# leggedrobotics/open3d_slam_private

Measured on AMD Instinct MI355X. Metric: ICP iterations/sec (scan-to-map), higher is better.
Workload: dtype f32

## Files before the change

open3d_slam_private_amd/csrc/host_loop.hpp:

```cpp
#pragma once


static reg_status check_ready(reg_handle* h, bool need_prepared) {
    if (!h) return REG_BAD_ARGUMENT;
    if (!h->device_ok) return REG_DEVICE_ERROR;
    if (h->m == 0) {
        h->err = "no reference set (reg_set_target)";
        return REG_NOT_CONFIGURED;
    }
    if (h->n == 0) {
        h->err = "no reading set (reg_set_source)";
        return REG_NOT_CONFIGURED;
    }
    if (need_prepared && !h->prepared) {
        h->err = "reg_prepare has not been called for this reading";
        return REG_NOT_CONFIGURED;
    }
    return REG_OK;
}

static reg_status prepare_rowmajor(reg_handle* h, const float* T_init_row, const float* c_override = nullptr,
                                   int64_t n_global = 0, const IterState* init_state = nullptr) {
    reg_status s = check_ready(h, false);
    if (s != REG_OK) return s;
// ... 27 lines not shown
    }
    pmark("centroid");
    PrepArgs pa;
    pa.sums = sums;
    pa.sums_to_clear = sums_next;
    pa.n = n_global > 0 ? n_global : n;
    pa.c_ref = make_float3(h->c_ref[0], h->c_ref[1], h->c_ref[2]);
    std::memcpy(pa.T_init.m, T_init_row, 64);
    pa.centre = p2pl ? 1 : 0;
    pa.use_override = c_override ? 1 : 0;
    pa.c_override = c_override ? make_float3(c_override[0], c_override[1], c_override[2]) : make_float3(0.f, 0.f, 0.f);
    pa.out = h->s_prep.as<PrepState>();
    pa.host_out = h->d_prep_host;
    h->prep_pending = true;
    StateInit si;
    si.dst = nullptr;
    if (init_state) {
        si.init = *init_state;
        si.dst = h->i_iter.as<IterState>();
    } else {
        std::memset(&si.init, 0, sizeof(si.init));
    }
    k_prepare_source<<<grid_for(n), 256, 0, h->stream>>>(
        h->s_raw.as<float>(), h->s_stride, (p2pl && h->has_snrm) ? h->s_nrm_raw.as<float>() : nullptr, h->s_nstride, n, pa,
        p2pl ? 1 : 0, h->perm, h->s_xyz.as<float4>(), (p2pl && h->has_snrm) ? h->s_nrm.as<float4>() : nullptr,
        h->i_hint.as<uint8_t>(), h->i_hist.as<uint32_t>(), h->i_acc.as<double>(), kAccRows * kSums, si,
        h->i_cache.as<float4>());
    if (h->prm.cost == REG_COST_GICP)
        k_pack_cov<<<grid_for(n), 256, 0, h->stream>>>(h->s_cov_raw.as<float>(), n, h->perm, h->s_cov.as<float4>());
    pmark("prepare_source");
    HIPCHK(h, hipGetLastError());
    h->prepared = true;
    h->match_launches = 0;
    h->have_match = false;
    h->pm_have_match = false;
    return REG_OK;
}


static reg_status build_iter_state(reg_handle* h, const float* T_row, int update, IterState* st) {
    std::memset(st, 0, sizeof(IterState));
    for (int i = 0; i < 16; ++i) {
        st->T[i] = T_row[i];
        st->Td[i] = (double)T_row[i];
    }
    st->chk = Checkers();
    st->chk.max_iter = h->prm.max_iter;
    st->chk.min_diff_rot = h->prm.min_diff_rot;
    st->chk.min_diff_trans = h->prm.min_diff_trans;
    st->chk.smooth_len = h->prm.smooth_len;
    st->chk.init(T_row);
    st->cost = h->prm.cost;
    st->fixed_iters = h->prm.fixed_iters;
    st->max_iter = h->prm.max_iter;
    st->update = update;
    st->gicp_rot_eps = h->prm.gicp_rot_eps;
    st->gicp_trans_eps = h->prm.gicp_trans_eps;
    st->gicp_stop_rule = h->prm.gicp_stop_rule;
    st->gicp_rel_fitness = h->prm.gicp_rel_fitness;
    st->gicp_rel_rmse = h->prm.gicp_rel_rmse;
    st->n_total = (float)(h->n_total_hint > 0 ? h->n_total_hint : h->n);
    st->band_lo = st->band_hi = INFINITY;
    st->limit_last = st->limit_prev = INFINITY;
    st->use_trim = (h->prm.cost == REG_COST_P2PL && h->prm.use_trimmed) ? 1 : 0;
    st->trim_ratio = h->prm.trim_ratio;
    st->band_cap = kBandCap;
// ... 27 lines not shown
    HIPCHK(h, hipEventRecord(h->ev_iter, h->stream));
    h->iter_copy_pending = true;
    return REG_OK;
}

static void prof_mark(reg_handle* h, int kind, bool start) {
    if (!h->profiling) return;
    hipEvent_t e;
    if (hipEventCreate(&e) != hipSuccess) return;
    (void)hipEventRecord(e, h->stream);
    h->prof_ev.push_back(e);
    if (start) h->prof_kind.push_back(kind);
}

template <class K, class... A>
static void launch_timed(reg_handle* h, int kind, K kernel, dim3 grid, dim3 block, A... args) {
    hipEvent_t e0 = nullptr, e1 = nullptr;
    if (!h->profiling || hipEventCreate(&e0) != hipSuccess || hipEventCreate(&e1) != hipSuccess) {
        if (e0) (void)hipEventDestroy(e0);
        hipLaunchKernelGGL(kernel, grid, block, 0, h->stream, args...);
        return;
    }
    hipExtLaunchKernelGGL(kernel, grid, block, 0, h->stream, e0, e1, 0, args...);
    h->prof_ev.push_back(e0);
    h->prof_ev.push_back(e1);
    h->prof_kind.push_back(kind);
}

static reg_status enqueue_match(reg_handle* h, bool zero_hist = false) {
    const bool trim = h->prm.cost == REG_COST_P2PL && h->prm.use_trimmed;
    if (trim && zero_hist) HIPCHK(h, hipMemsetAsync(h->i_hist.p, 0, 3 * 2048 * 4, h->stream));
    const bool fused_hist = h->dbg.match_variant == 3;
    uint32_t* hist0 = (trim && fused_hist) ? h->i_hist.as<uint32_t>() : nullptr;
    uint32_t* hist2 = trim ? h->i_hist.as<uint32_t>() + 4096 : nullptr;
    const IterState* it = h->i_iter.as<IterState>();
    if (h->dbg.match_variant == 1) {
        prof_mark(h, 0, true);
        k_match<<<h->n_blocks, 256, 0, h->stream>>>(h->s_xyz.as<float4>(), h->n, it, h->grid, h->i_pos.as<int>(),
                                                    h->i_d2.as<float>(), hist0, hist2, h->shift0);
        prof_mark(h, 0, false);
    } else {
        uint8_t* hint = h->dbg.match_variant == 2 ? nullptr : h->i_hint.as<uint8_t>();
        const int lanes = h->dbg.lanes_per_point == 4 ? 4 : (h->dbg.lanes_per_point == 2 ? 2 : 8);
        const int blocks = grid_for(h->n * lanes);
        const int tile = h->match_launches < 2 ? h->env.xcd_tile_first : h->env.xcd_tile_later;
        ++h->match_launches;
        const dim3 grid(xcd_tiled_grid(blocks, tile)), block(256);
        auto go = [&](auto kernel) {
            launch_timed(h, 0, kernel, grid, block, (const float4*)h->s_xyz.as<float4>(), h->n, it, h->grid,
                         h->i_pos.as<int>(), h->i_d2.as<float>(), hist0, hist2, hint, h->shift0, h->dbg.debug_flags, blocks,
                         h->i_cache.as<float4>(), tile);
        };
        if (lanes == 4)
            go(k_match_g8<4>);
        else if (lanes == 2)
            go(k_match_g8<2>);
        else
            go(k_match_g8<8>);
    }
    h->have_match = true;
    return REG_OK;
}

static reg_status enqueue_select(reg_handle* h) {
    uint32_t* hist0 = h->i_hist.as<uint32_t>();
    SelectState* st = h->i_state.as<SelectState>();
    const IterState* it = h->i_iter.as<IterState>();
    const int hb = std::min(h->n_blocks, 128);
    const float ratio = h->prm.trim_ratio;
    if (h->dbg.match_variant != 3)
        k_hist_level0<<<hb, 256, 0, h->stream>>>(h->i_d2.as<float>(), h->n, h->shift0, hist0, it);
    k_select_level<<<hb, 256, 0, h->stream>>>(h->i_d2.as<float>(), h->n, 1, h->shift0, ratio, hist0, hist0 + 2048,
                                              nullptr, st, it);
    k_select_level<<<hb, 256, 0, h->stream>>>(h->i_d2.as<float>(), h->n, 2, h->shift0, ratio, hist0 + 2048,
                                              hist0 + 4096, hist0, st, it);
    return REG_OK;
}

static FilterCfg make_filter_cfg(const reg_handle* h, int trim_mode);

static reg_status enqueue_linearize(reg_handle* h, bool want_w, bool limit_from_state = false) {
    float* w = want_w ? h->i_w.as<float>() : nullptr;
    const IterState* it = h->i_iter.as<IterState>();
    if (h->prm.cost == REG_COST_P2PL) {
        const FilterCfg f = make_filter_cfg(h, h->prm.use_trimmed ? (limit_from_state ? 1 : 2) : 0);
        k_linearize_p2pl<<<h->n_blocks, 256, 0, h->stream>>>(
            h->s_xyz.as<float4>(), h->has_snrm ? h->s_nrm.as<float4>() : nullptr, h->n, it, h->i_pos.as<int>(),
            h->i_d2.as<float>(), h->t_pts.as<float4>(), h->t_nrm.as<float4>(), f, h->i_state.as<SelectState>(),
            h->i_hist.as<uint32_t>() + 4096, h->i_hist.as<uint32_t>() + 2048, h->shift0, w,
            h->i_partials.as<double>(), h->i_cache.as<float4>());
    } else if (cost_is_o3d(h->prm.cost)) {
        const float3 o = make_float3(h->t_mid[0], h->t_mid[1], h->t_mid[2]);
        if (h->prm.cost == REG_COST_O3D_P2PL)
            k_linearize_o3d<REG_COST_O3D_P2PL><<<h->n_blocks, 256, 0, h->stream>>>(
                h->s_xyz.as<float4>(), h->n, it, h->i_pos.as<int>(), h->i_d2.as<float>(), h->t_nrm.as<float4>(), o, w,
                h->i_partials.as<double>());
        else
            k_linearize_o3d<REG_COST_O3D_P2P><<<h->n_blocks, 256, 0, h->stream>>>(
                h->s_xyz.as<float4>(), h->n, it, h->i_pos.as<int>(), h->i_d2.as<float>(), h->t_pts.as<float4>(), o, w,
                h->i_partials.as<double>());
        ++h->seq;
        k_reduce_update_o3d<<<1, 1024, 0, h->stream>>>(h->i_partials.as<double>(), h->n_blocks, h->i_iter.as<IterState>(),
                                                       h->d_mirror, h->seq);
        return REG_OK;
    } else {
        k_linearize_gicp<<<h->n_blocks, 256, 0, h->stream>>>(h->s_xyz.as<float4>(), h->s_cov.as<float4>(), h->n, it,
                                                             h->i_pos.as<int>(), h->i_d2.as<float>(),
                                                             h->t_pts.as<float4>(), h->t_cov.as<float4>(), w,
                                                             h->i_partials.as<double>());
    }
    ++h->seq;
    k_reduce_update<<<1, 1024, 0, h->stream>>>(h->i_partials.as<double>(), h->n_blocks, h->i_iter.as<IterState>(),
                                               h->d_mirror, h->seq, 0, nullptr, nullptr,
                                               h->prm.cost == REG_COST_P2PL ? h->i_state.as<SelectState>() : nullptr,
                                               nullptr, 0, 0, h->i_xicp.as<XicpState>());
    if (h->xicp_pending) {
        h->xicp_pending = false;
        const int blocks = (int)std::min<int64_t>(512, (h->n + 255) / 256);
        k_xicp_center<<<blocks, 256, 0, h->stream>>>(h->s_xyz.as<float4>(), h->n, h->i_iter.as<IterState>(),
                                                     h->i_pos.as<int>(), h->i_w.as<float>(), h->i_xicp.as<XicpState>());
        k_xicp_detect<<<blocks, 256, 0, h->stream>>>(h->s_xyz.as<float4>(), h->n, h->i_iter.as<IterState>(),
                                                     h->i_pos.as<int>(), h->i_w.as<float>(), h->t_nrm.as<float4>(),
                                                     h->i_xicp.as<XicpState>());
        k_reduce_update<<<1, 1024, 0, h->stream>>>(nullptr, 0, h->i_iter.as<IterState>(), h->d_mirror, h->seq, 2, nullptr,
                                                   nullptr, nullptr, nullptr, 0, 0, h->i_xicp.as<XicpState>());
    }
    return REG_OK;
}

static FilterCfg make_filter_cfg(const reg_handle* h, int trim_mode) {
    FilterCfg f;
    f.use_trim = trim_mode;
    f.use_normal = h->prm.use_surface_normal;
    f.use_maxdist = h->prm.use_max_dist_filter;
    f.debug = h->dbg.debug_flags;
    f.cos_max_angle = std::cos(h->prm.max_normal_angle);
    const float md = h->prm.outlier_max_dist;
    f.outlier_max_d2 = md * md;
    return f;
}

static inline float coherent_slack(const reg_handle* h) { return 0.25f * h->info.cell_size; }
static inline int coherent_search_grid(const reg_handle* h) { return (int)std::min<int64_t>(1024, (h->n + 31) / 32); }
static inline int coherent_queue_cap(int64_t n) { return (int)(((n + 255) / 256 + kQueues - 1) / kQueues) * 256; }

template <int G>
static void launch_fused(reg_handle* h, const FilterCfg& f, float* w, uint8_t* hint) {
    int blocks;
    if (h->dbg.debug_flags & 16) {
        blocks = grid_for(h->n * G);
        launch_timed(h, 1, k_iter_fused<G>, dim3(8 * ((blocks + 7) / 8)), dim3(256), (const float4*)h->s_xyz.as<float4>(),
                     (const float4*)(h->has_snrm ? h->s_nrm.as<float4>() : nullptr), h->n, h->i_iter.as<IterState>(), h->grid,
                     (const float4*)h->t_nrm.as<float4>(), f, h->i_pos.as<int>(), h->i_d2.as<float>(), w, hint,
                     h->i_band.as<float>(), (int)kBandCap, h->i_acc.as<double>(), blocks);
    } else {
        blocks = grid_for(h->n);
        launch_timed(h, 1, k_coh_check, dim3(8 * ((blocks + 7) / 8)), dim3(256), (const float4*)h->s_xyz.as<float4>(),
                     (const float4*)(h->has_snrm ? h->s_nrm.as<float4>() : nullptr), h->n, h->i_iter.as<IterState>(), h->grid,
                     (const float4*)h->t_nrm.as<float4>(), f, h->i_pos.as<int>(), h->i_d2.as<float>(), w,
                     (const float4*)h->i_cache.as<float4>(), h->i_queue.as<uint32_t>(), coherent_queue_cap(h->n),
// ... 127 lines not shown
    cfg.timeout_ticks = (unsigned long long)(h->env.tail_timeout_s * 1e8);
    float* w = want_w ? h->i_w.as<float>() : nullptr;
    uint8_t* hint = h->dbg.match_variant == 2 ? nullptr : h->i_hint.as<uint8_t>();
    hipEvent_t e0 = nullptr, e1 = nullptr;
    const bool timed = h->profiling && hipEventCreate(&e0) == hipSuccess && hipEventCreate(&e1) == hipSuccess;
    const bool gicp = h->prm.cost == REG_COST_GICP;
    auto args = [&](auto launch) {
        const float4* s_attr = gicp ? (const float4*)h->s_cov.as<float4>() : (const float4*)(h->has_snrm ? h->s_nrm.as<float4>() : nullptr);
        const float4* t_attr = gicp ? (const float4*)h->t_cov.as<float4>() : (const float4*)h->t_nrm.as<float4>();
        auto go = [&](auto kernel) {
            launch(kernel, dim3(pl.grid), dim3(kTailThreads), (const float4*)h->s_xyz.as<float4>(), s_attr, h->i_iter.as<IterState>(),
                   h->grid, t_attr, f, h->i_pos.as<int>(), h->i_d2.as<float>(), w, hint, h->i_cache.as<float4>(),
                   sync_cur, h->i_tail_rows.as<double>(), h->i_tail_band.as<float>(), h->d_mirror, cfg, sync_next);
        };
        if (gicp)
            go(k_tail<true>);
        else
            go(k_tail<false>);
    };
    if (timed) {
        args([&](auto k, dim3 g, dim3 b, auto... a) { hipExtLaunchKernelGGL(k, g, b, kTailLdsBytes, h->stream, e0, e1, 0, a...); });
        h->prof_ev.push_back(e0);
        h->prof_ev.push_back(e1);
        h->prof_kind.push_back(3);
    } else {
        if (e0) (void)hipEventDestroy(e0);
        args([&](auto k, dim3 g, dim3 b, auto... a) { hipLaunchKernelGGL(k, g, b, kTailLdsBytes, h->stream, a...); });
    }
    HIPCHK(h, hipGetLastError());
    h->have_match = true;
    return REG_OK;
}

static reg_status enqueue_iteration(reg_handle* h, bool want_w) {
    reg_status s = enqueue_match(h);
    if (s != REG_OK) return s;
    if (h->prm.cost == REG_COST_P2PL && h->prm.use_trimmed) {
        s = enqueue_select(h);
        if (s != REG_OK) return s;
    }
    return enqueue_linearize(h, want_w);
}

static inline unsigned long long mirror_seq(const reg_handle* h) {
    return __atomic_load_n(&h->h_mirror->seq, __ATOMIC_ACQUIRE);
}

static reg_status wait_seq(reg_handle* h, unsigned long long seq) {
    for (unsigned spins = 0;; ++spins) {
        if (mirror_seq(h) >= seq) return REG_OK;
        __builtin_ia32_pause();
        if ((spins & 0x3fff) == 0x3fff) {
            hipError_t e = hipStreamQuery(h->stream);
            if (e == hipSuccess) return REG_OK;
            if (e != hipErrorNotReady) {
                h->err = std::string("device fault while waiting for the iteration: ") + hipGetErrorString(e);
                return REG_DEVICE_ERROR;
            }
        }
    }
}

static reg_status iterate_once(reg_handle* h, const float* T_row, bool want_w) {
    reg_status s = init_iter_state(h, T_row, 0);
    if (s != REG_OK) return s;
    s = enqueue_iteration(h, want_w);
    if (s != REG_OK) return s;
    s = wait_seq(h, h->seq);
    if (s != REG_OK) return s;
// ... 517 lines not shown
    float T_start[16];
    if (p2pl)
        m4_identity(T_start);
    else
        std::memcpy(T_start, Ti, 64);
    std::memcpy(h->T_init, Ti, 64);
    IterState st0;
    reg_status s = build_iter_state(h, T_start, 1, &st0);
    if (s != REG_OK) return s;
    rmark("iter state");
    s = prepare_rowmajor(h, Ti, nullptr, 0, &st0);
    if (s != REG_OK) return s;
    rmark("prepared");
    h->profiling = h->dbg.profile_loop != 0;
    const bool event_timing = h->profiling || h->env.event_timing;
    if (event_timing) HIPCHK(h, hipEventRecord(h->ev0, h->stream));
    const auto t_loop_begin = std::chrono::steady_clock::now();
    rmark("ev0");
    const unsigned long long seq0 = h->seq;
    const int fixed = h->prm.fixed_iters;
    const int limit = sequence_limit(h->prm);
    const bool can_fuse = p2pl && h->dbg.disable_fused != 1;
    const bool trimming = p2pl && h->prm.use_trimmed && h->prm.trim_ratio != 1.0f;
    const int kGenericFirst = trimming ? 2 : (h->prm.cost == REG_COST_GICP ? std::max(1, h->env.gicp_tail_after) : 1);
    const int kAhead = h->env.lookahead;
    const HostMirror* mir = h->h_mirror;
    int generic_left = kGenericFirst;
    const bool trace = h->env.trace;
    float settle_tol = h->env.settle_tol;
    unsigned long long last_traced = 0;
    const auto t_loop0 = std::chrono::steady_clock::now();
    unsigned long long acked = seq0;
    int stalls = 0;
    const TailPlan tail_pl = ((can_fuse || h->prm.cost == REG_COST_GICP) && tail_eligible(h)) ? tail_plan(h) : TailPlan();
    const RegActiveGuard active(h->prm.device);
    std::unique_lock<std::mutex> tail_lock;
    if (tail_pl.ok && (active.alone() || h->env.tail_always)) {
        tail_lock = std::unique_lock<std::mutex>(g_tail_mutex[h->prm.device], std::try_to_lock);
    }
    const bool use_tail = tail_pl.ok && tail_lock.owns_lock();
    const int tail_min_iters = fixed > 0 ? 0 : h->env.tail_min_iters;
    const float fused_settle_tol = settle_tol;
    unsigned long long tail_seq = 0;
    bool tail_off = false;
    h->last_tail_launches = 0;
    h->last_tail_iters = 0;
    for (;;) {
        if (tail_seq) {
            for (unsigned spins = 0;; ++spins) {
                const unsigned long long m = mirror_seq(h);
                if (m >= tail_seq) break;
                if (m + 1 == tail_seq) {
                    const HostMirror::SeqRecord* rec = &mir->ring[(tail_seq - 1) % kSeqRing];
                    if (__atomic_load_n(&rec->seq, __ATOMIC_ACQUIRE) == tail_seq - 1 && (rec->done || rec->stall)) break;
                }
                __builtin_ia32_pause();
                if ((spins & 0xfff) == 0xfff) {
                    const hipError_t e = hipStreamQuery(h->stream);
                    if (e == hipSuccess) break;
                    if (e != hipErrorNotReady) {
                        h->tail_sync_dirty = true;
                        h->err = std::string("device fault while waiting for the tail kernel: ") + hipGetErrorString(e);
                        return REG_DEVICE_ERROR;
                    }
                }
            }
// ... 9 lines not shown
                return REG_DEVICE_ERROR;
            }
            if (!reported && !(mir->stall && std::max(mirror_seq(h), seq0) > acked)) acked = h->seq;
            if (h->env.coh_stats)
                fprintf(stderr, "[o3dreg] tail launch: %u iterations, %u point searches (%.2f %% of the point-iterations), stall cause %u, band records of its last iteration %d\n", words[2],
                        words[1], words[2] ? 100.0 * words[1] / ((double)words[2] * (double)h->n) : 0.0, words[3], reported ? mir->pad_nband : -1);
            if (reported) h->last_tail_iters += mir->pad3;
            if (reported && mir->stall && fixed <= 0) tail_off = true;
#if O3D_TAIL_STAMPS
            {
                unsigned long long st[24];
                (void)hipMemcpy(st, h->i_tail_sync.as<unsigned>() + (size_t)h->tail_sync_last * (kTailSyncBytes / 4) + kTailStampWord, sizeof(st),
                                 hipMemcpyDeviceToHost);
                const double it_n = std::max(1, reported ? mir->pad3 : 1);
                static const char* names[12] = {"check", "search", "epilogue", "bandrec+comps", "sum+publish+drain", "arrive+wait", "row sums",
                                                "band-stage", "band-scan", "band-rank", "band-add", "solve+update"};
                for (int wg = 0; wg < 2; ++wg) {
                    fprintf(stderr, "[o3dreg] tail stamps (us per iteration, %s workgroup):", wg ? "last" : "first");
                    for (int i = 0; i < 12; ++i) fprintf(stderr, " %s %.2f", names[i], st[12 * wg + i] * 0.01 / it_n);
                    fprintf(stderr, "\n");
                }
            }
#endif
            tail_seq = 0;
            continue;
        }
        const unsigned long long m_seq = std::max(mirror_seq(h), seq0);
        const bool any = m_seq > seq0;
        if (any && mir->done) break;
        if (any && mir->stall && m_seq > acked) {
            HIPCHK(h, hipStreamSynchronize(h->stream));
            acked = h->seq;
            generic_left = 2;
            ++stalls;
            continue;
        }
        if (trace && m_seq != last_traced) {
            last_traced = m_seq;
            float mt = 0.f, mr = 0.f;
            last_step_motion(mir, &mt, &mr);
            fprintf(stderr, "[o3dreg] seq %llu iter %d stall %d band_n %d limit %.6g prev %.6g band [%.6g, %.6g) step %.2e m %.2e rad\n",
                    m_seq - seq0, mir->iterations, mir->stall, mir->stall ? mir->band_count : mir->pad_nband, mir->limit_last, mir->limit_prev,
                    mir->band_lo, mir->band_hi, mt, mr);
        }
        acked = std::max(acked, m_seq);
        const int completed = any ? mir->iterations : 0;
        const int inflight = (int)(h->seq - acked);
        if (completed + inflight < limit && inflight < kAhead) {
            const bool tail_now = use_tail && !tail_off && completed + inflight >= tail_min_iters;
            settle_tol = tail_now ? h->env.tail_settle_tol : fused_settle_tol;
            bool settled = true;
            if (trimming) {
                settled = any && mir->limit_prev < INFINITY && mir->limit_last < INFINITY &&
                          std::fabs(mir->limit_last - mir->limit_prev) <= settle_tol * mir->limit_last;
            }
            if (settled && any && (p2pl || fixed <= 0) && (can_fuse || tail_now)) {
                float mt = 0.f, mr = 0.f;
                last_step_motion(mir, &mt, &mr);
                if (mt > h->env.settle_trans || mr > h->env.settle_rot) settled = false;
            }
            const auto tq0 = std::chrono::steady_clock::now();
            const bool go_generic = !(can_fuse || tail_now) || generic_left > 0 || !settled;
            if (go_generic) {
                s = enqueue_iteration(h, true);
                if (generic_left > 0) --generic_left;
            } else if (tail_now) {
                s = enqueue_tail(h, tail_pl, limit - (completed + inflight), true);
                tail_seq = h->seq;
                ++h->last_tail_launches;
            } else {
                int burst = fixed > 0 && !h->env.no_burst ? limit - (completed + inflight) : 1;
                for (; burst > 0 && s == REG_OK; --burst) s = enqueue_fused(h, true);
            }
            if (trace) {
                const auto tq1 = std::chrono::steady_clock::now();
                fprintf(stderr, "[o3dreg] t=%.1fus enqueue seq %llu (%s) took %.1fus; mirror at %llu\n",
                        std::chrono::duration<double, std::micro>(tq0 - t_loop0).count(), h->seq - seq0,
                        go_generic ? "generic" : (tail_now ? "tail" : "fused"), std::chrono::duration<double, std::micro>(tq1 - tq0).count(),
                        std::max(mirror_seq(h), seq0) - seq0);
            }
            if (s != REG_OK) return s;
            continue;
        }
        if (inflight == 0) break;
        s = wait_seq(h, acked + 1);
        if (s != REG_OK) return s;
        if (mirror_seq(h) <= acked) {
            if (hipStreamQuery(h->stream) == hipSuccess && mirror_seq(h) <= acked) acked = h->seq;
        }
    }
    h->last_stalls = stalls;
    rmark("loop done");
    if (event_timing) {
        HIPCHK(h, hipEventRecord(h->ev1, h->stream));
        HIPCHK(h, hipEventSynchronize(h->ev1));
        (void)hipEventElapsedTime(&res->loop_ms, h->ev0, h->ev1);
    } else {
        res->loop_ms = std::chrono::duration<float, std::milli>(std::chrono::steady_clock::now() - t_loop_begin).count();
// ... 610 lines not shown
```

open3d_slam_private_amd/csrc/host_target.hpp:

```cpp
#pragma once



struct DevBuf {
    void* p = nullptr;
    size_t cap = 0;
    hipError_t reserve(size_t bytes) {
        if (bytes <= cap) return hipSuccess;
        if (p) (void)hipFree(p);
        p = nullptr;
        cap = 0;
        hipError_t e = hipMalloc(&p, bytes ? bytes : 16);
        if (e == hipSuccess) cap = bytes;
        return e;
    }
    void release() {
        if (p) (void)hipFree(p);
        p = nullptr;
        cap = 0;
    }
    template <class T>
    T* as() const {
        return (T*)p;
    }
};

struct EnvSwitches {
    bool trace = false;
    bool event_timing = false;
    bool halo_occ = true;
    bool no_dynprune = false;
    bool no_empty_bound = false;
    bool no_burst = false;
    bool hints = false;
    bool stamps = false;
    bool coh_stats = false;
    bool tail_always = false;
    bool no_tail = false;
    int tail_wpc = 0;
    double dist_timeout_s = 30.0;
    float tail_timeout_s = 2.f;
    int xcd_tile_first = 32;
    int xcd_tile_later = 16;
    float settle_trans = 0.02f;
    float settle_rot = 4e-3f;
    int tail_min_iters = 8;
    int tail_tile = 0;
    bool no_gicp_tail = false;
    int gicp_tail_after = 1;
    float tail_settle_tol = 1.2f;
    int lookahead = 2;
    float settle_tol = 0.05f;
    float halo_ratio = 1.5f;
    float halo_rho = 0.4f;
    float reach_bins = 7.25f;
    float bin_occupancy = 8.f;
    float level_ratio = 2.0f;
    void read() {
        trace = getenv("O3D_TRACE") != nullptr;
        event_timing = getenv("O3D_EVENT_TIMING") != nullptr;
        no_burst = getenv("O3D_NO_BURST") != nullptr;
        no_dynprune = getenv("O3D_NO_DYNPRUNE") != nullptr;
        no_empty_bound = getenv("O3D_NO_EMPTY_BOUND") != nullptr;
        halo_occ = getenv("O3D_NO_HALO_OCC") == nullptr;
        hints = getenv("O3D_HINTS") != nullptr;
        stamps = getenv("O3D_STAMPS") != nullptr;
        coh_stats = getenv("O3D_COH_STATS") != nullptr;
        tail_always = getenv("O3D_TAIL_ALWAYS") != nullptr;
        no_tail = getenv("O3D_NO_TAIL") != nullptr;
        if (const char* v = getenv("O3D_TAIL_WPC")) tail_wpc = std::max(0, atoi(v));
        if (const char* v = getenv("O3D_DIST_TIMEOUT_S")) dist_timeout_s = std::max(0.5, atof(v));
        if (const char* v = getenv("O3D_TAIL_SETTLE")) tail_settle_tol = (float)atof(v);
        if (const char* v = getenv("O3D_NO_GICP_TAIL")) no_gicp_tail = atoi(v) != 0;
        if (const char* v = getenv("O3D_TAIL_TILE")) tail_tile = std::max(0, atoi(v));
        if (const char* v = getenv("O3D_TAIL_MIN_ITERS")) tail_min_iters = std::max(0, atoi(v));
        if (const char* v = getenv("O3D_SETTLE_TRANS")) settle_trans = (float)atof(v);
        if (const char* v = getenv("O3D_SETTLE_ROT")) settle_rot = (float)atof(v);
        if (const char* v = getenv("O3D_XCD_TILE_FIRST")) xcd_tile_first = std::max(0, atoi(v));
        if (const char* v = getenv("O3D_XCD_TILE_LATER")) xcd_tile_later = std::max(0, atoi(v));
        if (const char* v = getenv("O3D_GICP_TAIL_AFTER")) gicp_tail_after = atoi(v);
        if (const char* v = getenv("O3D_TAIL_TIMEOUT_S")) tail_timeout_s = std::min(30.f, std::max(0.01f, (float)atof(v)));
        if (const char* v = getenv("O3D_KAHEAD")) lookahead = std::max(1, atoi(v));
        if (const char* v = getenv("O3D_SETTLE")) settle_tol = (float)atof(v);
        if (const char* v = getenv("O3D_HALO_RATIO")) halo_ratio = std::min(4.0f, std::max(0.5f, (float)atof(v)));
        if (const char* v = getenv("O3D_HALO_RHO")) halo_rho = std::min(1.0f, std::max(0.05f, (float)atof(v)));
        if (const char* v = getenv("O3D_REACH_BINS")) reach_bins = std::max(1.0f, (float)atof(v));
        if (const char* v = getenv("O3D_BIN_OCC")) bin_occupancy = std::min(64.0f, std::max(1.0f, (float)atof(v)));
        if (const char* v = getenv("O3D_LEVEL_RATIO")) level_ratio = std::min(4.0f, std::max(1.2f, (float)atof(v)));
    }
};

struct DistCtx;

struct reg_handle {
    reg_params prm;
    reg_debug_params dbg;
    EnvSwitches env;
    std::string err;
    hipStream_t stream = nullptr;
    bool own_stream = false;
    bool device_ok = false;
    bool structure_only = false;
// ... 19 lines not shown
    bool has_tnrm = false, has_tcov = false;
    float c_ref[3] = {0, 0, 0};
    float t_mid[3] = {0, 0, 0};
    DevBuf t_raw, t_nrm_raw, t_cov_raw, t_centred, t_keys, t_keys2, t_vals, t_vals2, t_pts, t_nrm, t_cov, t_flags,
        t_scan, t_hash, t_cells, t_tmp, t_misc, t_dir, t_rows;
    Grid grid;
    reg_target_info info;
    float target_build_ms = 0.f;

    int64_t n = 0;
    bool has_snrm = false, has_scov = false, prepared = false;
    int64_t s_stride = 3, s_nstride = 3;
    float c_read[3] = {0, 0, 0};
    DevBuf s_raw, s_nrm_raw, s_cov_raw, s_xyz, s_nrm, s_cov, s_misc;
    float T_init[16];
    float T0[16];
    DevBuf i_pos, i_d2, i_w, i_hist, i_state, i_partials, i_sums, i_ids;
    HostMirror* h_mirror = nullptr;
    HostMirror* d_mirror = nullptr;
    IterState* h_iter = nullptr;
    DevBuf i_iter;
    unsigned long long seq = 0;
    DevBuf t_halo_start, t_halo_cursor, t_halo_pts, t_halo_dir, i_band, i_acc, i_cache, i_stats, i_queue, i_qcount;
    DevBuf s_prep;
    PrepState* h_prep = nullptr;
    PrepState* d_prep_host = nullptr;
    int cent_slot = 0;
    bool prep_pending = false;
    DevBuf i_hint, s_keys, s_keys2, s_perm, s_perm2, s_tmp, i_tmpf;
    const uint32_t* perm = nullptr;
    int last_stalls = 0;
    int64_t n_total_hint = 0;
    int match_launches = 0;
    int tail_sync_slot = 0, tail_sync_last = 0;
    bool tail_sync_dirty = true;
    int last_tail_launches = 0, last_tail_iters = 0;
    DevBuf i_tail_sync, i_tail_rows, i_tail_band;
    unsigned long long dist_seq0 = 0;
    DevBuf d_contrib, d_gathered;
    int dist_ranks = 0, dist_rank = 0;
    DistCtx* dist = nullptr;
    unsigned long long src_epoch = 0;
    std::vector<hipEvent_t> prof_ev;
    std::vector<int> prof_kind;
    bool profiling = false;
    int shift0 = 21;
    int n_blocks = 0;
    bool have_match = false;
    bool pm_on = false;
    reg_pm_chain pm;
    bool pm_have_match = false;
    DevBuf pm_pos, pm_d2, pm_w, pm_keys, pm_hist, pm_sel, pm_state, pm_partials;
    DevBuf pm_sorted, pm_sort_tmp, pm_var;
    size_t pm_sort_bytes = 0;
    DevBuf pm_xstate, pm_xrows, pm_xmeans, pm_xcov;
    PmExtraState pm_xhost;
    PmCovOut pm_cov_host;
    bool pm_x_valid = false;
    bool pm_cov_valid = false;
    float pm_cov_ms = 0.f;
    double pm_last_error = 0.0;
    bool xt_on = false;
    reg_ternary_xicp xt;
    DevBuf xt_state, xt_rows;
    XtState xt_host;
    bool xt_valid = false;
// ... 1271 lines not shown
```

open3d_slam_private_amd/csrc/kernels_fused.hpp:

```cpp
#pragma once

constexpr int kBandCap = 16384;
constexpr int kContribHdr = 128;
__host__ __device__ __forceinline__ int contrib_cap_for(int n_ranks) {
    return n_ranks <= 1 ? 8192 : (n_ranks == 2 ? 4096 : (n_ranks <= 4 ? 2048 : (n_ranks <= 8 ? 1024 : 512)));
}
__host__ __device__ __forceinline__ size_t contrib_floats(int cap) { return (size_t)kContribHdr + (size_t)cap * 32; }
constexpr int kAccRows = 64;
constexpr int kRec = 32;
__host__ __device__ __forceinline__ size_t band_at(int comp, size_t slot) { return slot * kRec + (size_t)comp; }

__device__ __forceinline__ void p2pl_products(float3 p, float4 q, float4 nn, float w, float* vals) {
    float F[6];
    float a = p.y * nn.z, b = p.z * nn.y;
    F[0] = a - b;
    a = p.z * nn.x; b = p.x * nn.z;
    F[1] = a - b;
    a = p.x * nn.y; b = p.y * nn.x;
    F[2] = a - b;
    F[3] = nn.x; F[4] = nn.y; F[5] = nn.z;
    const float dx = p.x - q.x, dy = p.y - q.y, dz = p.z - q.z;
    float r = dx * nn.x;
    float t2 = dy * nn.y;
    r = r + t2;
// ... 237 lines not shown
            float bb = nr.y * nt.y;
            float val = a + bb;
            a = nr.z * nt.z;
            val = val + a;
            if (val < f.cos_max_angle) w = 0.f;
        }
        cls = md2 < band_lo ? 0 : (md2 < band_hi ? 1 : 2);
        row[9] = 1.f;
        if (cls == 0) row[11] = 1.f;
        if (w != 0.f && cls == 0) {
            float a = p.y * nn.z, bq = p.z * nn.y;
            row[0] = a - bq;
            a = p.z * nn.x; bq = p.x * nn.z;
            row[1] = a - bq;
            a = p.x * nn.y; bq = p.y * nn.x;
            row[2] = a - bq;
            row[3] = nn.x; row[4] = nn.y; row[5] = nn.z;
            const float dx = p.x - tq.x, dy = p.y - tq.y, dz = p.z - tq.z;
            float r = dx * nn.x;
            float t2 = dy * nn.y;
            r = r + t2;
            t2 = dz * nn.z;
            r = r + t2;
            row[6] = r;
            row[7] = 1.f;
            row[8] = 1.f;
            row[10] = md2;
        }
        if (cls == 1) write_band_record(it, band, band_cap, p, tq, nn, w, md2, (int)q);
    }
    pos_io[q] = mpos;
    d2_out[q] = mpos >= 0 ? md2 : INFINITY;
    if (w_out) w_out[q] = (cls == 2) ? 0.f : w;
}

__device__ __forceinline__ double coh_component(const float* E, int rows, int comp) {
    double acc = 0.0;
    if (comp < 28) {
        const int ia = kProdCode.a[comp] >> 2, ic = kProdCode.c[comp] >> 2;
        for (int i = 0; i < rows; ++i) {
            const float v = E[i * kCohRow + ia] * E[i * kCohRow + ic];
            acc += (double)v;
        }
    } else {
        const int ia = 8 + (comp - 28);
        for (int i = 0; i < rows; ++i) acc += (double)E[i * kCohRow + ia];
    }
    return acc;
}

__global__ void __launch_bounds__(256)
k_coh_check(const float4* __restrict__ src, const float4* __restrict__ src_nrm, int64_t n, IterState* __restrict__ it,
            Grid g, const float4* __restrict__ tgt_nrm, FilterCfg f, int* __restrict__ pos_io, float* __restrict__ d2_out,
            float* __restrict__ w_out, const float4* __restrict__ cache ,
            uint32_t* __restrict__ queue, int queue_cap, float* __restrict__ band, int band_cap, double* __restrict__ partials,
            int n_blocks) {
    __shared__ __attribute__((aligned(16))) float E[256 * kCohRow];
    __shared__ int s_wave_cnt[4];
    __shared__ unsigned s_base;
    __shared__ double sh[4][kSums];
    const int t = threadIdx.x;
    const int lb = xcd_block(n_blocks);
    const int64_t q = lb < n_blocks ? (int64_t)lb * 256 + t : n;
    const int64_t qc = q < n ? q : n - 1;
    const float4 s = src[qc];
    const float4 c = cache[qc];
// ... 203 lines not shown
```

open3d_slam_private_amd/csrc/kernels_update.hpp:

```cpp
#pragma once

__global__ void __launch_bounds__(64)
k_pack_contrib(double* __restrict__ acc, const IterState* __restrict__ it, float* __restrict__ contrib) {
    const int c = threadIdx.x;
    double* hdr = reinterpret_cast<double*>(contrib);
    if (it->done || it->stall) {
        if (c < kSums) hdr[c] = 0.0;
        if (c == 0) reinterpret_cast<uint32_t*>(contrib)[64] = 0u;
        return;
    }
    if (c < kSums) {
        double t = 0;
        for (int r = 0; r < kAccRows; ++r) {
            t += acc[(size_t)r * kSums + c];
            acc[(size_t)r * kSums + c] = 0.0;
        }
        hdr[c] = t;
    }
    if (c == 0) reinterpret_cast<uint32_t*>(contrib)[64] = it->band_count;
}

__device__ __forceinline__ void lds_barrier() {
    asm volatile("s_waitcnt lgkmcnt(0)" ::: "memory");
    __builtin_amdgcn_s_barrier();
// ... 99 lines not shown
        for (int b0 = part; b0 < n_rows; b0 += 32 * 8) {
            double v8[8];
#pragma unroll
            for (int u = 0; u < 8; ++u) {
                const int b = b0 + 32 * u;
                v8[u] = partials[(size_t)(b < n_rows ? b : part) * kSums + comp];
            }
#pragma unroll
            for (int u = 0; u < 8; ++u) t += (b0 + 32 * u < n_rows) ? v8[u] : 0.0;
        }
    }
    constexpr int kSpec = 6;
    const bool spec = fused == 1 && !gathered && band != nullptr;
    uint32_t spec_d2 = 0;
    int spec_idx = 0;
    float spec_pre[kSpec];
#pragma unroll
    for (int u = 0; u < kSpec; ++u) spec_pre[u] = 0.f;
    if (spec) {
        spec_d2 = __float_as_uint(band[band_at(29, threadIdx.x)]);
        if (w_out) spec_idx = __float_as_int(band[band_at(31, threadIdx.x)]);
        if (comp != 29 && comp != 31) {
#pragma unroll
            for (int u = 0; u < kSpec; ++u) spec_pre[u] = band[band_at(comp, (uint32_t)part + 32u * u)];
        }
    }
    __syncthreads();
    const int s_done = sit->done, s_stall = sit->stall, s_use_trim = sit->use_trim;
    const float s_ratio = sit->trim_ratio, s_band_lo = sit->band_lo, s_band_hi = sit->band_hi;
    uint32_t s_band_count = sit->band_count;
    bool band_bad = false;
    if (s_done) return;
    if (fused && s_stall) return;
    const unsigned long long st0 = __builtin_amdgcn_s_memtime();
    if (gathered) {
        if (threadIdx.x == 0) {
            uint32_t off = 0, bad = 0;
            for (int r = 0; r < n_ranks; ++r) {
                rk_off[r] = off;
                const uint32_t cnt = reinterpret_cast<const uint32_t*>(gathered + (size_t)r * contrib_stride)[64];
                if (cnt > (uint32_t)contrib_cap) bad = 1;
                off += min(cnt, (uint32_t)contrib_cap);
            }
            rk_off[n_ranks] = off;
            if (off > (uint32_t)kBandCap) bad = 1;
            rk_bad = bad;
        }
        __syncthreads();
        s_band_count = rk_off[n_ranks];
        band_bad = rk_bad != 0;
    }
    if (!gathered && s_band_count > (uint32_t)kBandCap) band_bad = true;
    auto rec = [&](uint32_t i, int c) -> float {
        if (!gathered) return band[band_at(c, i)];
        int r = 0;
        while (r + 1 < n_ranks && i >= rk_off[r + 1]) ++r;
        return gathered[(size_t)r * contrib_stride + kContribHdr + (size_t)(i - rk_off[r]) * kRec + c];
    };
    const bool trim = s_use_trim && s_ratio != 1.0f;
    const uint32_t n_band = (fused && trim && !band_bad) ? s_band_count : 0u;
    const bool add_comp = comp != 29 && comp != 31;
    constexpr int kPre = 8;
    float pre[kPre];
    uint32_t my_d2[1];
    if (n_band) {
        my_d2[0] = 0u;
// ... 545 lines not shown
```

Measured before the change: 16500.

## Add band-select path replacing second select level with fused band linearize

Adds a generic-iteration path for trimmed point-to-plane ICP. It runs only the level-0 and level-1 histogram selects, then a new k_linearize_band kernel. That kernel classifies each point as below, inside or above the trim band, accumulates the normal equations for points below the band, and records in-band points for k_reduce_update to resolve. This removes the level-2 select kernel and the separate linearize pass per iteration, and hist0 is zeroed inside the kernel instead of by a memset. The path falls back to the classic route for a couple of iterations after each stall and is disabled if the band overflows kBandCap, at the cost of more state bookkeeping and an extra xicp_stage check in the reduce kernel.

```diff
diff --git a/open3d_slam_private_amd/csrc/host_loop.hpp b/open3d_slam_private_amd/csrc/host_loop.hpp
--- a/open3d_slam_private_amd/csrc/host_loop.hpp
+++ b/open3d_slam_private_amd/csrc/host_loop.hpp
@@ -83,6 +83,8 @@
     HIPCHK(h, hipGetLastError());
     h->prepared = true;
     h->match_launches = 0;
+    h->hist_dirty = 2;
+    h->select_band_off = false;
     h->have_match = false;
     h->pm_have_match = false;
     return REG_OK;
@@ -176,7 +178,8 @@
     if (trim && zero_hist) HIPCHK(h, hipMemsetAsync(h->i_hist.p, 0, 3 * 2048 * 4, h->stream));
     const bool fused_hist = h->dbg.match_variant == 3;
     uint32_t* hist0 = (trim && fused_hist) ? h->i_hist.as<uint32_t>() : nullptr;
-    uint32_t* hist2 = trim ? h->i_hist.as<uint32_t>() + 4096 : nullptr;
+    uint32_t* hist2 = trim ? h->i_hist.as<uint32_t>() + 2048 * h->hist_dirty : nullptr;
+    h->hist_dirty = 2;
     const IterState* it = h->i_iter.as<IterState>();
     if (h->dbg.match_variant == 1) {
         prof_mark(h, 0, true);
@@ -222,6 +225,7 @@
 }
 
 static FilterCfg make_filter_cfg(const reg_handle* h, int trim_mode);
+static void enqueue_xicp_first(reg_handle* h);
 
 static reg_status enqueue_linearize(reg_handle* h, bool want_w, bool limit_from_state = false) {
     float* w = want_w ? h->i_w.as<float>() : nullptr;
@@ -258,6 +262,11 @@
                                                h->d_mirror, h->seq, 0, nullptr, nullptr,
                                                h->prm.cost == REG_COST_P2PL ? h->i_state.as<SelectState>() : nullptr,
                                                nullptr, 0, 0, h->i_xicp.as<XicpState>());
+    enqueue_xicp_first(h);
+    return REG_OK;
+}
+
+static void enqueue_xicp_first(reg_handle* h) {
     if (h->xicp_pending) {
         h->xicp_pending = false;
         const int blocks = (int)std::min<int64_t>(512, (h->n + 255) / 256);
@@ -269,7 +278,6 @@
         k_reduce_update<<<1, 1024, 0, h->stream>>>(nullptr, 0, h->i_iter.as<IterState>(), h->d_mirror, h->seq, 2, nullptr,
                                                    nullptr, nullptr, nullptr, 0, 0, h->i_xicp.as<XicpState>());
     }
-    return REG_OK;
 }
 
 static FilterCfg make_filter_cfg(const reg_handle* h, int trim_mode) {
@@ -463,9 +471,36 @@
     return REG_OK;
 }
 
-static reg_status enqueue_iteration(reg_handle* h, bool want_w) {
+static bool select_band_usable(const reg_handle* h) {
+    return h->prm.cost == REG_COST_P2PL && h->prm.use_trimmed && h->dbg.disable_fused != 1 && !(h->dbg.debug_flags & (1 | 2 | 4)) &&
+           !h->env.no_select_band && !h->select_band_off;
+}
+static reg_status enqueue_select_band(reg_handle* h, bool want_w) {
+    uint32_t* const hist0 = h->i_hist.as<uint32_t>();
+    SelectState* st = h->i_state.as<SelectState>();
+    IterState* it = h->i_iter.as<IterState>();
+    const int hb = std::min(h->n_blocks, 128);
+    if (h->dbg.match_variant != 3) k_hist_level0<<<hb, 256, 0, h->stream>>>(h->i_d2.as<float>(), h->n, h->shift0, hist0, it);
+    k_select_level<<<hb, 256, 0, h->stream>>>(h->i_d2.as<float>(), h->n, 1, h->shift0, h->prm.trim_ratio, hist0, hist0 + 2048,
+                                              nullptr, st, it);
+    const FilterCfg f = make_filter_cfg(h, 0);
+    float* w = want_w ? h->i_w.as<float>() : nullptr;
+    k_linearize_band<<<h->n_blocks, 256, 0, h->stream>>>(
+        h->s_xyz.as<float4>(), h->has_snrm ? h->s_nrm.as<float4>() : nullptr, h->n, it, h->i_pos.as<int>(), h->i_d2.as<float>(),
+        h->t_nrm.as<float4>(), f, st, hist0 + 2048, hist0, h->shift0, w, h->i_band.as<float>(), (int)kBandCap,
+        h->i_acc.as<double>(), h->i_cache.as<float4>());
+    h->hist_dirty = 1;
+    ++h->seq;
+    k_reduce_update<<<1, 1024, 0, h->stream>>>(h->i_acc.as<double>(), h->n_blocks, it, h->d_mirror, h->seq, 1, h->i_band.as<float>(),
+                                               w, nullptr, nullptr, 0, 0, h->i_xicp.as<XicpState>());
+    enqueue_xicp_first(h);
+    return REG_OK;
+}
+
+static reg_status enqueue_iteration(reg_handle* h, bool want_w, bool band = false) {
     reg_status s = enqueue_match(h);
     if (s != REG_OK) return s;
+    if (band && select_band_usable(h)) return enqueue_select_band(h, want_w);
     if (h->prm.cost == REG_COST_P2PL && h->prm.use_trimmed) {
         s = enqueue_select(h);
         if (s != REG_OK) return s;
@@ -1049,6 +1084,7 @@
     const auto t_loop0 = std::chrono::steady_clock::now();
     unsigned long long acked = seq0;
     int stalls = 0;
+    int classic_left = 0;
     const TailPlan tail_pl = ((can_fuse || h->prm.cost == REG_COST_GICP) && tail_eligible(h)) ? tail_plan(h) : TailPlan();
     const RegActiveGuard active(h->prm.device);
     std::unique_lock<std::mutex> tail_lock;
@@ -1124,6 +1160,9 @@
             HIPCHK(h, hipStreamSynchronize(h->stream));
             acked = h->seq;
             generic_left = 2;
+            classic_left = 2;
+            if ((unsigned)mir->band_count > (unsigned)kBandCap) h->select_band_off = true;
+            if (mir->iterations == 0 && h->prm.use_xicp && p2pl) h->xicp_pending = true;
             ++stalls;
             continue;
         }
@@ -1154,8 +1193,9 @@
             const auto tq0 = std::chrono::steady_clock::now();
             const bool go_generic = !(can_fuse || tail_now) || generic_left > 0 || !settled;
             if (go_generic) {
-                s = enqueue_iteration(h, true);
+                s = enqueue_iteration(h, true, classic_left == 0);
                 if (generic_left > 0) --generic_left;
+                if (classic_left > 0) --classic_left;
             } else if (tail_now) {
                 s = enqueue_tail(h, tail_pl, limit - (completed + inflight), true);
                 tail_seq = h->seq;
diff --git a/open3d_slam_private_amd/csrc/host_target.hpp b/open3d_slam_private_amd/csrc/host_target.hpp
--- a/open3d_slam_private_amd/csrc/host_target.hpp
+++ b/open3d_slam_private_amd/csrc/host_target.hpp
@@ -36,6 +36,7 @@
     bool stamps = false;
     bool coh_stats = false;
     bool tail_always = false;
+    bool no_select_band = false;
     bool no_tail = false;
     int tail_wpc = 0;
     double dist_timeout_s = 30.0;
@@ -68,6 +69,7 @@
         coh_stats = getenv("O3D_COH_STATS") != nullptr;
         tail_always = getenv("O3D_TAIL_ALWAYS") != nullptr;
         no_tail = getenv("O3D_NO_TAIL") != nullptr;
+        no_select_band = getenv("O3D_NO_SELECT_BAND") != nullptr;
         if (const char* v = getenv("O3D_TAIL_WPC")) tail_wpc = std::max(0, atoi(v));
         if (const char* v = getenv("O3D_DIST_TIMEOUT_S")) dist_timeout_s = std::max(0.5, atof(v));
         if (const char* v = getenv("O3D_TAIL_SETTLE")) tail_settle_tol = (float)atof(v);
@@ -153,6 +155,8 @@
     int last_stalls = 0;
     int64_t n_total_hint = 0;
     int match_launches = 0;
+    int hist_dirty = 2;
+    bool select_band_off = false;
     int tail_sync_slot = 0, tail_sync_last = 0;
     bool tail_sync_dirty = true;
     int last_tail_launches = 0, last_tail_iters = 0;
diff --git a/open3d_slam_private_amd/csrc/kernels_fused.hpp b/open3d_slam_private_amd/csrc/kernels_fused.hpp
--- a/open3d_slam_private_amd/csrc/kernels_fused.hpp
+++ b/open3d_slam_private_amd/csrc/kernels_fused.hpp
@@ -293,6 +293,131 @@
     pos_io[q] = mpos;
     d2_out[q] = mpos >= 0 ? md2 : INFINITY;
     if (w_out) w_out[q] = (cls == 2) ? 0.f : w;
+}
+
+__global__ void __launch_bounds__(256)
+k_linearize_band(const float4* __restrict__ src, const float4* __restrict__ src_nrm, int64_t n, IterState* __restrict__ it,
+                 const int* __restrict__ pos, const float* __restrict__ d2, const float4* __restrict__ tgt_nrm, FilterCfg f,
+                 const SelectState* __restrict__ st, const uint32_t* __restrict__ hist1, uint32_t* __restrict__ hist0_to_zero,
+                 int shift0, float* __restrict__ w_out, float* __restrict__ band, int band_cap,
+                 double* __restrict__ acc, float4* __restrict__ cache ) {
+    __shared__ uint32_t wave_tot[4];
+    __shared__ uint32_t pick[3];
+    __shared__ double sh[4][kSums];
+    const int64_t i = blockIdx.x * (int64_t)blockDim.x + threadIdx.x;
+    const int64_t ic = i < n ? i : n - 1;
+    const int ps_raw = pos[ic];
+    const float dd = d2[ic];
+    const float4 s = src[ic];
+    const float4 sn = *(f.use_normal ? src_nrm + ic : src + ic);
+    uint32_t loc[8];
+    load_hist8(hist1, loc);
+    const int st_done = it->done, st_stall = it->stall;
+    const float ratio = it->trim_ratio;
+    const Xf T = load_xf(it);
+    const uint32_t st_nfin = st->n_finite, st_prefix = st->prefix, st_rank = st->rank;
+#pragma unroll
+    for (int k = 0; k < 12; ++k) asm volatile("" ::"s"(T.m[k]));
+    asm volatile("" ::"s"(st_nfin), "s"(st_prefix), "s"(st_rank), "s"(ratio));
+    asm volatile("" ::"v"(ps_raw), "v"(dd), "v"(s.x), "v"(sn.x), "v"(loc[0]), "v"(loc[4]));
+    if (st_done) return;
+    if (blockIdx.x == 0)
+        for (int k = threadIdx.x; k < 2048; k += blockDim.x) hist0_to_zero[k] = 0;
+    if (st_stall) return;
+    const int ps = i < n ? ps_raw : -1;
+    const int psc = ps >= 0 ? ps : 0;
+    const float4 nn_ld = tgt_nrm[2 * (size_t)psc + 1];
+    const float4 q_ld = tgt_nrm[2 * (size_t)psc];
+    uint32_t u_lo = 0x7f800000u, u_hi = 0x7f800000u;
+    if (ratio != 1.0f && st_nfin != 0) {
+        block_pick256_regs(loc, st_rank, wave_tot, pick);
+        u_lo = st_prefix | (pick[0] << (shift0 - 11));
+        u_hi = u_lo + (1u << (shift0 - 11));
+    }
+    if (blockIdx.x == 0 && threadIdx.x == 0) {
+        it->band_lo = __uint_as_float(u_lo);
+        it->band_hi = __uint_as_float(u_hi);
+    }
+    float w = 0.f;
+    int cls = 2;
+    float3 p = make_float3(0.f, 0.f, 0.f);
+    if (ps >= 0) {
+        w = 1.f;
+        if (f.use_maxdist && !(dd <= f.outlier_max_d2)) w = 0.f;
+        p = xf_point(T, s.x, s.y, s.z);
+        if (f.use_normal) {
+            const float3 nr = normalize3(xf_rot(T, sn.x, sn.y, sn.z));
+            const float3 nt = normalize3(make_float3(nn_ld.x, nn_ld.y, nn_ld.z));
+            float a = nr.x * nt.x;
+            float b = nr.y * nt.y;
+            float val = a + b;
+            a = nr.z * nt.z;
+            val = val + a;
+            if (val < f.cos_max_angle) w = 0.f;
+        }
+        const uint32_t u = __float_as_uint(dd);
+        cls = u < u_lo ? 0 : (u < u_hi ? 1 : 2);
+        if (cls == 1) write_band_record(it, band, band_cap, p, q_ld, nn_ld, w, dd, (int)i);
+    }
+    double v[kSums];
+#pragma unroll
+    for (int k = 0; k < kSums; ++k) v[k] = 0.0;
+    if (ps >= 0) {
+        v[29] = 1.0;
+        if (cls == 0) v[31] = 1.0;
+        if (w != 0.f && cls == 0) {
+            const float4 nn = nn_ld, q = q_ld;
+            float F[6];
+            float a = p.y * nn.z, b = p.z * nn.y;
+            F[0] = a - b;
+            a = p.z * nn.x; b = p.x * nn.z;
+            F[1] = a - b;
+            a = p.x * nn.y; b = p.y * nn.x;
+            F[2] = a - b;
+            F[3] = nn.x; F[4] = nn.y; F[5] = nn.z;
+            const float dx = p.x - q.x, dy = p.y - q.y, dz = p.z - q.z;
+            float r = dx * nn.x;
+            float t2 = dy * nn.y;
+            r = r + t2;
+            t2 = dz * nn.z;
+            r = r + t2;
+            int k = 0;
+#pragma unroll
+            for (int a6 = 0; a6 < 6; ++a6) {
+                const float wf = w * F[a6];
+#pragma unroll
+                for (int c6 = a6; c6 < 6; ++c6) {
+                    const float pr = wf * F[c6];
+                    v[k++] = (double)pr;
+                }
+            }
+#pragma unroll
+            for (int a6 = 0; a6 < 6; ++a6) {
+                const float wf = w * F[a6];
+                const float pr = wf * r;
+                v[21 + a6] = (double)pr;
+            }
+            const float rr = r * r;
+            v[27] = (double)(w * rr);
+            v[28] = 1.0;
+            v[30] = (double)dd;
+        }
+    }
+    if (i < n) {
+        if (w_out) w_out[i] = cls == 2 ? 0.f : w;
+        if (cache && ps >= 0) {
+            cache[(size_t)n + i] = q_ld;
+            cache[2 * (size_t)n + i] = make_float4(nn_ld.x, nn_ld.y, nn_ld.z, 1.f);
+        }
+    }
+    const int lane = threadIdx.x & 63, wave = threadIdx.x >> 6;
+    wave_reduce32(v);
+    if ((lane & 1) == 0) sh[wave][lane >> 1] = v[0];
+    __syncthreads();
+    if (threadIdx.x < kSums) {
+        const double t = (sh[0][threadIdx.x] + sh[1][threadIdx.x]) + (sh[2][threadIdx.x] + sh[3][threadIdx.x]);
+        unsafeAtomicAdd(&acc[(size_t)(blockIdx.x & (kAccRows - 1)) * kSums + threadIdx.x], t);
+    }
 }
 
 __device__ __forceinline__ double coh_component(const float* E, int rows, int comp) {
diff --git a/open3d_slam_private_amd/csrc/kernels_update.hpp b/open3d_slam_private_amd/csrc/kernels_update.hpp
--- a/open3d_slam_private_amd/csrc/kernels_update.hpp
+++ b/open3d_slam_private_amd/csrc/kernels_update.hpp
@@ -155,6 +155,7 @@
     bool band_bad = false;
     if (s_done) return;
     if (fused && s_stall) return;
+    if (finish && sit->xicp_stage != 2) return;
     const unsigned long long st0 = __builtin_amdgcn_s_memtime();
     if (gathered) {
         if (threadIdx.x == 0) {
```

After: 16420. Within noise of the previous version (-0.5%).
